# wangyunpeng139/3_ORB_SLAM3_SelfNote

Hardware: AMD Instinct MI355X
Metric: frames/sec ORB extract+match, 752x480 (higher is better)
Workload: dtype u8; 1 GPU; BASELINE configs[2]: extract + SearchByProjection match, 1000x1000 candidates, synthetic frame stream; image=752x480, nfeatures=1000, nlevels=8, batch=256, distinct_frames_per_gpu=2048, streams=4

## Files before the change

3_orb_slam3_selfnote_amd/csrc/orb_common.h:

```cpp
#pragma once
#include <stdint.h>
#include <stddef.h>

#define ORB_EDGE_THRESHOLD 19
#define ORB_PATCH_SIZE 31
#define ORB_HALF_PATCH 15
#define ORB_MIN_BORDER 16
#define ORB_DISC_PIXELS 749
#define ORB_MAXL 16

#define FAST_TILE_PITCH 80
#define FAST_TILE_COLS 65
#define FAST_TILE_ROWS 76
#define FAST_S_PITCH 64

#define FAST_REC_WORDS 32
#define FAST_REC_GROUP_WORDS 8
#define FAST_REC_CELL_WORDS 4

#ifndef ORB_DESCRIBE_K
#define ORB_DESCRIBE_K 8
#endif
#define ORB_DESCRIBE_GROUPS(totalKp, K) ((((totalKp) + (K) - 1) / (K) + 3) / 4 > 1 ? (((totalKp) + (K) - 1) / (K) + 3) / 4 : 1)

__host__ __device__ constexpr int clamp_count(int n, int cap) { return (n > 0 ? n : 0) < cap ? (n > 0 ? n : 0) : cap; }
static_assert(clamp_count(-1, 8) == 0 && clamp_count(0, 8) == 0 && clamp_count(5, 8) == 5 && clamp_count(8, 8) == 8 && clamp_count(9, 8) == 8, "clamp_count");
static_assert(clamp_count(-1, 0) == 0 && clamp_count(0, 0) == 0 && clamp_count(1, 0) == 0, "clamp_count: cap == 0");

struct LiveCount {
  const int32_t *dev; int stride; int konst;
  __device__ __forceinline__ int at(int p, int cap) const { return dev ? clamp_count(dev[(size_t)p * stride], cap) : konst; }
};

// ... 7 lines not shown
  int nCols, nRows, wCell, hCell;
  int cellCap;
  int cellBase;
  int slotBase;
  int N;
  int nIni;
  float hX;
  int candBase;
  int candCap;
  int kpBase, kpCap;
  float scale;
  float kpsize;
  int xtabBase, ytabBase;
  int resizeRows;
  int resizeSrcRows;
  int tilesX, tilesY, tileBase;
  uint32_t rowTileMagic;
};

#define CHAIN_TILE 32
#define CHAIN_NT 1024
struct ChainTile {
  uint16_t level, pad;
  uint16_t x[ORB_MAXL], y[ORB_MAXL], w[ORB_MAXL], h[ORB_MAXL];
};

struct FrameParams {
  LevelGeom geom[ORB_MAXL];
  int nlevels;
  int nframes;
// ... 8 lines not shown
  uint32_t *cand;    int cand_fs;
  uint16_t *knode;
  uint32_t *lkp;     int lkp_fs;
  uint16_t *lrank;
  int32_t *lcnt;
  int32_t *candCnt;
  const int2 *xtab, *ytab;
  const int8_t *disc;
  const uint32_t *tiles;
  uint32_t magicCells, magicTiles, magicKpBlk;
  int totalTiles;
  int totalCells;
  int totalGroups;
  uint32_t magicGroups;
  const uint32_t *fastRecs;
  int totalKp;
  int octCap;
  const ChainTile *chain;
  int chainBuf0, chainBuf1;
  void *out_kps;
  uint8_t *out_desc;
  int32_t *out_counts;
  int cap;
};
```

3_orb_slam3_selfnote_amd/csrc/orb_kernels.h:

```cpp
#pragma once
#include <hip/hip_runtime.h>
#include <type_traits>
#include "orb_common.h"
#include "orb_fast_score.h"
#include "orb_sincos.h"

#define WAVE 64

__constant__ __attribute__((aligned(16))) int8_t c_pattern[1024] = {
#include "../../include/orb_pattern_data.inc"
};

struct DiscTab { uint32_t w[64][6]; };
constexpr int kDiscUmax[16] = {15, 15, 15, 15, 14, 14, 14, 13, 13, 12, 11, 10, 9, 8, 6, 3};
constexpr DiscTab make_disc_tab() {
  DiscTab t{};
  int n = 0;
  for (int v = -15; v <= 15; v++) {
    const int d = kDiscUmax[v < 0 ? -v : v];
    for (int u = -d; u <= d; u++) {
      const int lane = n & 63, k = n >> 6;
      t.w[lane][k >> 2] |= (uint32_t)(uint8_t)(int8_t)u << (8 * (k & 3));
      t.w[lane][3 + (k >> 2)] |= (uint32_t)(uint8_t)(int8_t)v << (8 * (k & 3));
      n++;
// ... 77 lines not shown
    uint32_t inc = wave_incl_scan(v);
    if (lane == 63) sw[wid] = inc;
    __syncthreads();
    const uint32_t wsum = lane < NW ? sw[lane] : 0u;
    const uint32_t wincl = wave_incl_scan(wsum);
    const int widu = __builtin_amdgcn_readfirstlane(wid);
    const uint32_t woff = (uint32_t)__builtin_amdgcn_readlane((int)(wincl - wsum), widu);
    const uint32_t tot = (uint32_t)__builtin_amdgcn_readlane((int)wincl, NW - 1);
    if (i < n) a[i] = carry + woff + inc - v;
    carry += tot;
    __syncthreads();
  }
  return carry;
}

#define RESIZE_ROWS_MAX 16
#define RESIZE_MAXSRC 32
__global__ __launch_bounds__(256) void k_resize(FrameParams P, int level, int smemRowBytes, int tPitch, int maxSrc) {
  extern __shared__ __align__(16) uint8_t smem_rs[];
  const LevelGeom G = P.geom[level];
  const LevelGeom Gs = P.geom[level - 1];
  const int tid = threadIdx.x;
  int frame, rowTile;
  xcd_map((G.h + G.resizeRows - 1) / G.resizeRows, G.rowTileMagic, P.nframes, frame, rowTile);
  const int dy0 = rowTile * G.resizeRows;
  const int nrows = min(G.resizeRows, G.h - dy0);
  int spitch;
  const uint8_t *src = level_plane(P, frame, level - 1, spitch);
  uint8_t *dstplane = P.pyr + (size_t)frame * P.pyr_fs + G.off;
  const int wq = (G.w + 3) & ~3, qw = wq >> 2;
  __shared__ int2 sY[RESIZE_ROWS_MAX];
  if (tid < nrows) sY[tid] = P.ytab[G.ytabBase + dy0 + tid];

  if (tPitch > 0) {
    const int syFirst = min(max(P.ytab[G.ytabBase + dy0].x, 0), Gs.h - 1);
    const int syLast = min(max(P.ytab[G.ytabBase + dy0 + nrows - 1].x + 1, 0), Gs.h - 1);
    const int nsrc = min(syLast - syFirst + 1, maxSrc);
    uint8_t *sRows = smem_rs;
    uint8_t *sT = sRows + (size_t)maxSrc * smemRowBytes;
    uint4 *sRowRec = reinterpret_cast<uint4 *>(sT + (((size_t)maxSrc * tPitch + 15) & ~(size_t)15));
    const int4 *xtab4 = reinterpret_cast<const int4 *>(P.xtab + G.xtabBase);
    int4 xtPre[2];
#pragma unroll
    for (int k = 0; k < 2; k++) { const int p = tid + 256 * k; xtPre[k] = 2 * p < wq ? xtab4[p] : make_int4(0, 0, 0, 0); }
    const bool aligned = ((((uintptr_t)src) | (uintptr_t)spitch) & 3u) == 0;
    const uint8_t *src0 = src + (size_t)syFirst * spitch;
    if (aligned) {
      const int cpr = smemRowBytes >> 4, nfull = Gs.w >> 4;
      const float inv_cpr = 1.0f / (float)cpr;
      for (int idx = tid; idx < cpr * nsrc; idx += 256) {
        const int r = (int)(((float)idx + 0.5f) * inv_cpr), c = idx - (int)mul24((uint32_t)r, (uint32_t)cpr);
        if (c < nfull)
          __builtin_amdgcn_global_load_lds((const __attribute__((address_space(1))) void *)(src0 + (mul24((uint32_t)r, (uint32_t)spitch) + 16u * (uint32_t)c)),
                                           (__attribute__((address_space(3))) void *)(sRows + (size_t)(idx - (tid & 63)) * 16), 16, 0, 0);
      }
      const int ndw = (Gs.w + 3) >> 2, d0 = 4 * nfull, ntail = ndw - d0;
      const bool lastRowPartial = (Gs.w & 3) != 0;
      for (int idx = tid; idx < ntail * nsrc; idx += 256) {
        const int r = idx / ntail, d = d0 + (idx - r * ntail);
// ... 2 lines not shown
        if (lastRowPartial && d == ndw - 1 && syFirst + r == Gs.h - 1 && spitch < 4 * ndw) {
          v = 0;
          for (int b = 0; 4 * d + b < Gs.w; b++) v |= (uint32_t)rowp[4 * d + b] << (8 * b);
        } else {
          v = *reinterpret_cast<const uint32_t *>(rowp + 4 * d);
        }
        *reinterpret_cast<uint32_t *>(sRows + mul24((uint32_t)r, (uint32_t)smemRowBytes) + 4 * d) = v;
      }
    } else {
      const float inv_w = 1.0f / (float)Gs.w;
      for (int idx = tid; idx < Gs.w * nsrc; idx += 256) {
        const int r = (int)(((float)idx + 0.5f) * inv_w), c = idx - (int)mul24((uint32_t)r, (uint32_t)Gs.w);
        sRows[mul24((uint32_t)r, (uint32_t)smemRowBytes) + c] = src0[mul24((uint32_t)r, (uint32_t)spitch) + c];
      }
    }
    if (tid < nrows) {
      const int2 yt = P.ytab[G.ytabBase + dy0 + tid];
      const int sy0 = min(max(yt.x, 0), Gs.h - 1), sy1 = min(max(yt.x + 1, 0), Gs.h - 1);
      sRowRec[tid] = make_uint4((uint32_t)((sy0 - syFirst) * tPitch), (uint32_t)((sy1 - syFirst) * tPitch), (uint32_t)yt.y, (uint32_t)((dy0 + tid) * G.pitch));
    }
    __syncthreads();
    typedef unsigned short u16x2 __attribute__((ext_vector_type(2)));
    auto dot2 = [](uint32_t pix, uint32_t coef) -> uint32_t {
      u16x2 x, y;
      __builtin_memcpy(&x, &pix, 4); __builtin_memcpy(&y, &coef, 4);
      return __builtin_amdgcn_udot2(x, y, 0u, false);
    };
    int trip = 0;
    for (int p = tid; 2 * p < wq; p += 256, trip++) {
      const int4 xt = trip == 0 ? xtPre[0] : trip == 1 ? xtPre[1] : xtab4[p];
      const uint32_t base = (uint32_t)xt.x & ~3u, oA = (uint32_t)xt.x & 3u, oB = (uint32_t)xt.z - base;
      const uint32_t selA = 0x0c000c00u | oA | ((oA + 1u) << 16), selB = 0x0c000c00u | oB | ((oB + 1u) << 16);
      const uint32_t kA = (uint32_t)xt.y << 4, kB = (uint32_t)xt.w << 4;
      const uint8_t *sp = sRows + base;
      uint8_t *tp = sT + 4 * p;
      for (int r = 0; r < nsrc; r += 4) {
// ... 20 lines not shown
      for (int qx = tid & 31; qx < qw; qx += 32) {
        const uint2 t0 = *reinterpret_cast<const uint2 *>(T0 + 8 * qx), t1 = *reinterpret_cast<const uint2 *>(T1 + 8 * qx);
        const uint32_t u0[4] = {t0.x & 0xffffu, t0.x >> 16, t0.y & 0xffffu, t0.y >> 16};
        const uint32_t u1[4] = {t1.x & 0xffffu, t1.x >> 16, t1.y & 0xffffu, t1.y >> 16};
        uint32_t packed = 0;
#pragma unroll
        for (int j = 0; j < 4; j++) {
          const uint32_t v = ((mul24_vv(b0, u0[j]) >> 16) + (mul24_vv(b1, u1[j]) >> 16) + 2) >> 2;
          packed |= v << (8 * j);
        }
        const int dx0 = 4 * qx;
        if (dx0 + 3 < G.w) *reinterpret_cast<uint32_t *>(dst + dx0) = packed;
        else for (int j = 0; j < 4 && dx0 + j < G.w; j++) dst[dx0 + j] = (uint8_t)(packed >> (8 * j));
      }
    }
    return;
  }

  int2 *sX = reinterpret_cast<int2 *>(smem_rs);
  for (int i = tid; i < wq; i += 256) sX[i] = P.xtab[G.xtabBase + i];
  __syncthreads();
  const float inv_qw = 1.0f / (float)qw;
  for (int q = tid; q < qw * nrows; q += 256) {
    const int ry = (int)(((float)q + 0.5f) * inv_qw), dx0 = (q - (int)mul24((uint32_t)ry, (uint32_t)qw)) * 4, dy = dy0 + ry;
    const int2 yt = sY[ry];
    const int sy0 = min(max(yt.x, 0), Gs.h - 1), sy1 = min(max(yt.x + 1, 0), Gs.h - 1);
    const int b0 = yt.y & 0xffff, b1 = (yt.y >> 16) & 0xffff;
    const uint8_t *S0 = src + mul24((uint32_t)sy0, (uint32_t)spitch), *S1 = src + mul24((uint32_t)sy1, (uint32_t)spitch);
    uint32_t packed = 0;
#pragma unroll
    for (int j = 0; j < 4; j++) {
      const int2 xt = sX[dx0 + j];
      const int sx = xt.x, sx1 = min(sx + 1, Gs.w - 1);
      const int a0 = xt.y & 0xffff, a1 = (xt.y >> 16) & 0xffff;
      const int r0 = S0[sx] * a0 + S0[sx1] * a1;
      const int r1 = S1[sx] * a0 + S1[sx1] * a1;
      const int v = (((b0 * (r0 >> 4)) >> 16) + ((b1 * (r1 >> 4)) >> 16) + 2) >> 2;
      packed |= (uint32_t)v << (8 * j);
    }
    uint8_t *dst = dstplane + mul24((uint32_t)dy, (uint32_t)G.pitch);
    if (dx0 + 3 < G.w) *reinterpret_cast<uint32_t *>(dst + dx0) = packed;
    else for (int j = 0; j < 4 && dx0 + j < G.w; j++) dst[dx0 + j] = (uint8_t)(packed >> (8 * j));
  }
}

__global__ __launch_bounds__(CHAIN_NT) void k_pyramid_chain(FrameParams P) {
  extern __shared__ __align__(16) uint8_t smem_ch[];
  const int tid = threadIdx.x, lane = tid & 63, wid = tid >> 6;
  constexpr int NW = CHAIN_NT / 64;
  const int ntile = (int)gridDim.x / P.nframes;
  const int frame = (int)blockIdx.x / ntile, tile = (int)blockIdx.x - frame * ntile;
  __shared__ ChainTile T;
  static_assert(sizeof(ChainTile) % 4 == 0 && sizeof(ChainTile) / 4 <= CHAIN_NT, "one dword per thread");
  if (tid < (int)(sizeof(ChainTile) / 4)) reinterpret_cast<uint32_t *>(&T)[tid] = reinterpret_cast<const uint32_t *>(&P.chain[tile])[tid];
  __syncthreads();
  const int L = T.level;
  uint8_t *buf[2] = {smem_ch, smem_ch + P.chainBuf0};
  int2 *sTab = reinterpret_cast<int2 *>(smem_ch + P.chainBuf0 + P.chainBuf1);
// ... 53 lines not shown
  const int B = (int)(uint16_t)min((uint16_t)max(p0, p8), (uint16_t)max(p4, p12));
  return (D - (v - t)) | ((v + t) - B);
}

#ifndef FAST_NT
#define FAST_NT 256
#endif
#define FAST_QUEUE 128
#ifndef FAST_LIST
#define FAST_LIST 384
#endif
static_assert(FAST_NT == 4 * WAVE, "k_fast gives each cell of a 2 x 2 group a wavefront of its own");
static_assert(FAST_LIST % WAVE == 0, "pass 3 reads the corner list 64 entries at a time, all inside the list");
static_assert((FAST_TILE_ROWS * FAST_TILE_PITCH) % 16 == 0, "the score plane is cleared in 16-byte stores");
static_assert(FAST_TILE_ROWS * FAST_TILE_PITCH <= 65536, "queue entries are 16-bit tile offsets");
#if defined(FAST_STAMPS) || defined(OCT_STAMPS)
__device__ unsigned int *g_fast_stamps;
#endif
#ifdef FAST_STAMPS
#define FSTAMP(i) do { const long long t_ = __builtin_readcyclecounter(); if (threadIdx.x == 0 && g_fast_stamps) g_fast_stamps[(size_t)blockIdx.x * 8 + (i)] = (unsigned int)(t_ - ft0); ft0 = t_; } while (0)
#else
#define FSTAMP(i) do {} while (0)
#endif
__device__ __forceinline__ void wave_lds_order() {
  __builtin_amdgcn_wave_barrier();
  asm volatile("" ::: "memory");
}
__global__ __launch_bounds__(FAST_NT) void k_fast(FrameParams P) {
#ifdef FAST_STAMPS
  long long ft0 = __builtin_readcyclecounter();
#endif
  __shared__ __align__(16) uint8_t sTile[FAST_TILE_ROWS * FAST_TILE_PITCH];
  __shared__ __align__(16) uint8_t sS[FAST_TILE_ROWS * FAST_TILE_PITCH];
// ... 542 lines not shown
        t.v[lane][8 + 4 * s + d] = vv;
      }
  }
  return t;
}
__device__ const BlurTab g_blurTab = make_blur_tab();

#define BLUR_TX 128
#ifndef BLUR_TY
#define BLUR_TY 64
#endif
#define BLUR_ROWS_IN (BLUR_TY + 6)
#define BLURM_PITCH 176
#define BLURM_OPITCH 144
__global__ __launch_bounds__(256) __attribute__((amdgpu_waves_per_eu(7, 7))) void k_blur(FrameParams P) {
  typedef int v4i __attribute__((ext_vector_type(4)));
  typedef int v16i __attribute__((ext_vector_type(16)));
  __shared__ __align__(16) uint8_t sLds[BLUR_ROWS_IN * BLURM_PITCH + BLUR_TY * BLURM_OPITCH];
  static_assert(BLUR_TY % 32 == 0 && (BLUR_TY + 32) * BLURM_PITCH <= BLUR_ROWS_IN * BLURM_PITCH + BLUR_TY * BLURM_OPITCH, "the last block's rows must stay inside the allocation");
  uint8_t *sIn = sLds, *sOut = sLds + BLUR_ROWS_IN * BLURM_PITCH;
  const int tid = threadIdx.x, lane = tid & 63, wid = tid >> 6;
  int tile, frame;
  xcd_map(P.totalTiles, P.magicTiles, P.nframes, frame, tile);
  const uint4 t0 = reinterpret_cast<const uint4 *>(P.tiles)[2 * tile], t1 = reinterpret_cast<const uint4 *>(P.tiles)[2 * tile + 1];
  const int x0 = (int)(t0.x & 0xffffu), y0 = (int)(t0.x >> 16), level = (int)t0.y;
  struct { int w, h, bpitch; size_t boff; } G;
  G.w = (int)(t0.z & 0xffffu); G.h = (int)(t0.z >> 16); G.bpitch = (int)(t0.w >> 16);
  G.boff = ((size_t)t1.w << 32) | t1.z;
  int pitch;
  const uint8_t *img;
  if (level == 0) { pitch = (int)P.img0_stride; img = P.img0 + (size_t)frame * P.img0_frame_stride; }
  else { pitch = (int)(t0.w & 0xffffu); img = P.pyr + (size_t)frame * P.pyr_fs + (((size_t)t1.y << 32) | t1.x); }
  const bool aligned = ((((uintptr_t)img) | (uintptr_t)pitch) & 3u) == 0;
  const int wlim = level == 0 ? G.w : pitch;
  const bool dma = aligned && G.w >= 160 && G.h >= 40 && (wlim & 15) == 0;
  const bool edgeL = x0 == 0, edgeR = x0 + 131 >= G.w;
  if (dma) {
    for (int idx = tid; idx < BLUR_ROWS_IN * 11; idx += 256) {
      const uint32_t r = mul24((uint32_t)idx, 5958u) >> 16, c = (uint32_t)idx - 11u * r;
      int yy = y0 - 3 + (int)r;
      yy = yy < 0 ? -yy : yy;
      yy = yy >= G.h ? 2 * (G.h - 1) - yy : yy;
      yy = max(yy, 0);
      int xb = x0 - 16 + 16 * (int)c;
      xb = min(max(xb, 0), wlim - 16);
      __builtin_amdgcn_global_load_lds((const __attribute__((address_space(1))) void *)(img + (mul24((uint32_t)yy, (uint32_t)pitch) + (uint32_t)xb)),
                                       (__attribute__((address_space(3))) void *)(sIn + idx * 16), 16, 0, 0);
    }
    if (edgeL || edgeR) {
      __syncthreads();
      for (int i = tid; i < BLUR_ROWS_IN * 6; i += 256) {
        const int r = (int)(mul24((uint32_t)i, 10923u) >> 16), k = i - 6 * r;
        const int x = k < 3 ? -1 - k : G.w + (k - 3);
        const int xs = k < 3 ? 1 + k : G.w - 2 - (k - 3);
        const bool need = k < 3 ? edgeL : (edgeR && x - (x0 - 16) < 160);
        if (need) sIn[r * BLURM_PITCH + (x - (x0 - 16))] = sIn[r * BLURM_PITCH + (xs - (x0 - 16))];
      }
    }
  } else {
    const bool small = G.w < 16 || G.h < 16;
    auto srcRow = [&](int r) {
      int yy = y0 + r - 3;
      if (small) yy = reflect101(yy, G.h);
// ... 6 lines not shown
      const uint8_t *row = srcRow((int)r);
      uint32_t v;
      if (aligned && xb >= 0 && xb + 3 < G.w) v = *reinterpret_cast<const uint32_t *>(row + xb);
      else {
        v = 0;
#pragma unroll
        for (int kk = 0; kk < 4; kk++) {
          int xx = xb + kk;
          if (small) xx = reflect101(xx, G.w);
          else { xx = xx < 0 ? -xx : xx; xx = xx >= G.w ? 2 * (G.w - 1) - xx : xx; xx = max(xx, 0); }
          v |= (uint32_t)row[xx] << (8 * kk);
        }
      }
      *reinterpret_cast<uint32_t *>(sIn + r * BLURM_PITCH + 4u * c) = v;
    }
  }
  const int n = lane & 31, hh = lane >> 5;
  v4i Hb[2], Va[2];
  {
    const uint4 *tab = reinterpret_cast<const uint4 *>(g_blurTab.v[lane]);
    const uint4 q0 = tab[0], q1 = tab[1], q2 = tab[2], q3 = tab[3];
    Hb[0] = v4i{(int)q0.x, (int)q0.y, (int)q0.z, (int)q0.w}; Hb[1] = v4i{(int)q1.x, (int)q1.y, (int)q1.z, (int)q1.w};
    Va[0] = v4i{(int)q2.x, (int)q2.y, (int)q2.z, (int)q2.w}; Va[1] = v4i{(int)q3.x, (int)q3.y, (int)q3.z, (int)q3.w};
  }
  __syncthreads();
  auto row_sums = [&](int mt, v4i &Bhi, v4i &Blo) {
    int seedT = 128 * 257;
    asm volatile("" : "+v"(seedT));
    v16i acc;
#pragma unroll
    for (int j = 0; j < 16; j++) acc[j] = seedT;
#pragma unroll
    for (int s = 0; s < 2; s++) {
      v4i a = *reinterpret_cast<const v4i *>(sIn + (32 * mt + n) * BLURM_PITCH + 32 * wid + 32 * s + 16 * hh);
      a[0] ^= (int)0x80808080; a[1] ^= (int)0x80808080; a[2] ^= (int)0x80808080; a[3] ^= (int)0x80808080;
      acc = __builtin_amdgcn_mfma_i32_32x32x32_i8(a, Hb[s], acc, 0, 0, 0);
    }
#pragma unroll
    for (int d = 0; d < 4; d++) {
      const uint32_t p01 = __builtin_amdgcn_perm((uint32_t)acc[4 * d + 1], (uint32_t)acc[4 * d], 0x05010400u);
// ... 17 lines not shown
      sOut[(row0 + (j & 3) + 8 * (j >> 2) + 4 * hh) * BLURM_OPITCH + 32 * wid + n] = (uint8_t)b;
    }
  };
  v4i Hp, Lp, Hc, Lc;
  row_sums(0, Hp, Lp);
#pragma unroll
  for (int k = 0; k < BLUR_TY / 32; k++) {
    if (k > 0 && y0 + 32 * k >= G.h) break;
    __builtin_amdgcn_sched_barrier(0);
    row_sums(k + 1, Hc, Lc);
    __builtin_amdgcn_sched_barrier(0);
    outputs(Hp, Lp, Hc, Lc, 32 * k);
    Hp = Hc; Lp = Lc;
  }
  __syncthreads();
#pragma unroll
  for (int t = 0; t < BLUR_TY / 32; t++) {
    const int row = (tid >> 3) + 32 * t, seg = tid & 7;
    const int y = y0 + row, x = x0 + 16 * seg;
    if (y < G.h && x < G.w) {
      uint8_t *out = P.blur + (size_t)frame * P.blur_fs + G.boff + (size_t)y * G.bpitch + x;
      const uint4 v = *reinterpret_cast<const uint4 *>(sOut + row * BLURM_OPITCH + 16 * seg);
      if (x + 16 <= G.bpitch) *reinterpret_cast<uint4 *>(out) = v;
      else {
        const uint8_t *b = sOut + row * BLURM_OPITCH + 16 * seg;
        for (int cc = 0; cc < 16 && x + cc < G.w; cc++) out[cc] = b[cc];
      }
    }
  }
}

__device__ __forceinline__ float fast_atan2_deg(float y, float x) {
  const float scale = (float)(180.0 / 3.1415926535897932384626433832795);
  const float p1 = 0.9997878412794807f * scale, p3 = -0.3258083974640975f * scale;
  const float p5 = 0.1555786518463281f * scale, p7 = -0.04432655554792128f * scale;
  float ax = fabsf(x), ay = fabsf(y);
  float a, c, c2;
  if (ax >= ay) {
    c = ay / (ax + (float)2.2204460492503131e-16);
    c2 = c * c;
    a = (((p7 * c2 + p5) * c2 + p3) * c2 + p1) * c;
  } else {
    c = ax / (ay + (float)2.2204460492503131e-16);
    c2 = c * c;
// ... 696 lines not shown
```

3_orb_slam3_selfnote_amd/csrc/orbhip.hip:

```cpp
#include <hip/hip_runtime.h>
#include <math.h>
#include <cmath>
#include <assert.h>
#include <stdio.h>
#include <stdlib.h>
#include <string.h>
#include <string>
#include <vector>
#include <algorithm>
#include <type_traits>
#include <mutex>
#include <map>
#include <chrono>

#include "../../include/orbhip.h"
#include "orb_kernels.h"
#include "orb_match_kernels.h"
#include "orb_match_mfma.h"
#include "orb_project_kernels.h"
#include "orb_stereo_kernels.h"
#include "orb_depth_kernels.h"
#include "orb_rig_stereo_kernels.h"
#include "orb_newpoints_kernels.h"
#include "orb_fuse_kernels.h"
// ... 45 lines not shown
  int device = 0;
  int nfeatures = 0, nlevels = 0, iniThFAST = 0, minThFAST = 0;
  double scaleFactor = 0;
  std::vector<float> mvScaleFactor, mvInvScaleFactor, mvLevelSigma2, mvInvLevelSigma2;
  std::vector<int> mnFeaturesPerLevel;
  int umax[ORB_HALF_PATCH + 1];
  int rows = 0, cols = 0, max_batch = 0;
  std::vector<LevelGeom> geom;
  size_t pyr_fs = 0, blur_fs = 0, slot_fs = 0;
  bool octCellsLds = false;
  int chainTiles = 0, chainBuf0 = 0, chainBuf1 = 0;
  size_t chainLds = 0;
  size_t octLds = 0;
  int cell_fs = 0, cand_fs = 0, lkp_fs = 0, totalTiles = 0, totalCells = 0, totalGroups = 0, totalKp = 0, octCap = 0;
  int maxKeypoints = 0;
  DevBuf d_pyr, d_blur, d_cellCnt, d_cellOff, d_slots, d_cand, d_knode, d_lkp, d_lrank, d_lcnt, d_candCnt, d_fastRecs, d_tiles, d_xtab,
      d_ytab, d_disc, d_chain;
  DevBuf d_img, d_okps;
  hipStream_t stream = nullptr;
  float host_us[4] = {0, 0, 0, 0};
  FrameParams last{};
  bool have_last = false;
  hipEvent_t last_done = nullptr;
  bool last_pending = false;
  bool in_capture = false;
  DevBuf stereo[7];
  DevBuf stereo_batch[3];
  DevBuf maps[2];
  int maps_rows = 0, maps_cols = 0;
  void *pin_in = nullptr, *pin_out = nullptr;
  size_t pin_in_bytes = 0, pin_out_bytes = 0;
// ... 163 lines not shown
  if (hipStreamCreateWithFlags(&h->stream, hipStreamNonBlocking) != hipSuccess) { delete h; return nullptr; }
  if (h->d_disc.reserve(disc.size()) != hipSuccess ||
      copy_on(h->stream, h->d_disc.p, disc.data(), disc.size(), hipMemcpyHostToDevice) != hipSuccess) {
    (void)hipStreamDestroy(h->stream);
    delete h;
    return nullptr;
  }
  return h;
}

void orbx_destroy(orbx_t *h) {
  if (!h) return;
  (void)hipSetDevice(h->device);
  if (h->stream) (void)hipStreamSynchronize(h->stream);
  DevBuf *bufs[] = {&h->d_pyr, &h->d_blur, &h->d_cellCnt, &h->d_cellOff, &h->d_slots, &h->d_cand, &h->d_knode, &h->d_lkp,
                    &h->d_lrank, &h->d_lcnt, &h->d_candCnt, &h->d_fastRecs, &h->d_tiles, &h->d_xtab, &h->d_ytab, &h->d_disc, &h->d_chain, &h->d_img, &h->d_okps};
  for (DevBuf *b : bufs) b->release();
  for (DevBuf &b : h->stereo) b.release();
  for (DevBuf &b : h->stereo_batch) b.release();
  for (DevBuf &b : h->maps) b.release();
  if (h->graph) (void)hipGraphExecDestroy(h->graph);
  if (h->last_done) (void)hipEventDestroy(h->last_done);
  if (h->pin_in) (void)hipHostFree(h->pin_in);
  if (h->pin_pyr) (void)hipHostFree(h->pin_pyr);
  h->d_pyrpack.release();
  if (h->pin_out) (void)hipHostFree(h->pin_out);
  if (h->ev_ok)
    for (auto &set : h->ev)
      for (auto &e : set) (void)hipEventDestroy(e);
  if (h->stream) (void)hipStreamDestroy(h->stream);
  delete h;
// ... 10 lines not shown
    if (isf) isf[i] = h->mvInvScaleFactor[i];
    if (s2) s2[i] = h->mvLevelSigma2[i];
    if (is2) is2[i] = h->mvInvLevelSigma2[i];
  }
  return h->nlevels;
}

int orbx_get_features_per_level(const orbx_t *h, int *n) {
  if (!h || !n) return ORBX_E_ARG;
  for (int i = 0; i < h->nlevels; i++) n[i] = h->mnFeaturesPerLevel[i];
  return h->nlevels;
}

static uint32_t magic_div(uint32_t n) { return n <= 1 ? 0xffffffffu : (uint32_t)((1ull << 32) / n); }

#if defined(FAST_STAMPS) || defined(OCT_STAMPS)
int orbx_debug_fast_stamps(void *d_buf) {
  unsigned int *p = (unsigned int *)d_buf;
  return hipMemcpyToSymbol(HIP_SYMBOL(g_fast_stamps), &p, sizeof(p)) == hipSuccess ? 0 : -1;
}
#endif

int orbx_max_keypoints(const orbx_t *h) { return h ? h->maxKeypoints : ORBX_E_ARG; }

int orbx_configure(orbx_t *h, int rows, int cols, int max_batch) {
  if (!h || rows <= 0 || cols <= 0 || max_batch <= 0) return ORBX_E_ARG;
  if (rows > 4096 || cols > 4096) { h->err = "image larger than 4096x4096 (12-bit packed coordinates)"; return ORBX_E_ARG; }
  if (max_batch > 65535) { h->err = "batch larger than 65535"; return ORBX_E_ARG; }
  if (h->rows == rows && h->cols == cols && h->max_batch >= max_batch) return h->maxKeypoints;
  XCHECK(h, hipSetDevice(h->device));
  XCHECK(h, hipStreamSynchronize(h->stream));
  const int nl = h->nlevels;
  std::vector<LevelGeom> g(nl);
  std::vector<int2> xtab, ytab;
  size_t pyr = 0, blur = 0;
  int cells = 0, slots = 0, kps = 0, tiles = 0, octCap = 8;
  for (int l = 0; l < nl; l++) {
    LevelGeom &G = g[l];
    memset(&G, 0, sizeof(G));
    const float inv = h->mvInvScaleFactor[l];
    G.w = cv_round((float)cols * inv);
    G.h = cv_round((float)rows * inv);
    if (G.w < 1 || G.h < 1) { h->err = "pyramid level collapses to zero size"; return ORBX_E_ARG; }
    G.pitch = (int)align_up((size_t)G.w, 64);
    G.bpitch = G.pitch;
    G.off = pyr;
    if (l > 0) pyr += align_up((size_t)G.pitch * G.h, 256);
    G.boff = blur;
    blur += align_up((size_t)G.bpitch * G.h, 256);
// ... 63 lines not shown
        ytab.push_back(make_int2(sy, (b0 & 0xffff) | (b1 << 16)));
      }
      auto src_rows = [&](int rows) {
        int m = 0;
        for (int dy0 = 0; dy0 < G.h; dy0 += rows) {
          const int nrows = std::min(rows, G.h - dy0);
          const int f = std::min(std::max(ytab[G.ytabBase + dy0].x, 0), sh - 1), la = std::min(std::max(ytab[G.ytabBase + dy0 + nrows - 1].x + 1, 0), sh - 1);
          m = std::max(m, la - f + 1);
        }
        return m;
      };
      const size_t rowStage = align_up((size_t)sw + 4, 16) + align_up((size_t)((G.w + 3) & ~3) * 2, 8);
      G.resizeRows = RESIZE_ROWS_MAX;
      G.resizeSrcRows = src_rows(G.resizeRows);
      if ((size_t)G.resizeSrcRows * rowStage > 64 * 1024 || G.resizeSrcRows > RESIZE_MAXSRC) { G.resizeRows = 8; G.resizeSrcRows = src_rows(8); }
    } else { G.resizeRows = RESIZE_ROWS_MAX; G.resizeSrcRows = 0; }
  }
  if (slots > (1 << 30)) { h->err = "workspace too large"; return ORBX_E_ARG; }
  std::vector<uint32_t> cellrec((size_t)std::max(cells, 1) * 4, 0u);
  for (int l = 0; l < nl; l++) {
    LevelGeom &G = g[l];
    G.rowTileMagic = magic_div((uint32_t)((G.h + G.resizeRows - 1) / G.resizeRows));
    for (int ci = 0; ci < G.nRows; ci++)
      for (int cj = 0; cj < G.nCols; cj++) {
        const int c = ci * G.nCols + cj;
        uint32_t *R = &cellrec[(size_t)(G.cellBase + c) * 4];
        const int iniX = ORB_MIN_BORDER + cj * G.wCell, iniY = ORB_MIN_BORDER + ci * G.hCell;
        const int maxX = std::min(iniX + G.wCell + 6, G.maxBorderX), maxY = std::min(iniY + G.hCell + 6, G.maxBorderY);
        const int tw = maxX - iniX, th = maxY - iniY;
        const bool valid = !(iniX >= G.maxBorderX - 6 || iniY >= G.maxBorderY - 3 || tw - 6 <= 0 || th - 6 <= 0);
// ... 42 lines not shown
            C[1] = R[1];
            C[2] = R[2];
            C[3] = (uint32_t)cell;
          }
      }
  }
  h->totalGroups = (int)(grouprec.size() / FAST_REC_WORDS);
  std::vector<uint32_t> tilerec((size_t)std::max(tiles, 1) * 8, 0u);
  for (int l = 0; l < nl; l++) {
    const LevelGeom &G = g[l];
    if (G.pitch > 65535 || G.bpitch > 65535) { h->err = "level pitch above 65535"; return ORBX_E_ARG; }
    if (l > 0 && (size_t)((G.w + 3) & ~3) * 8 > ORB_LDS_LIMIT - 1024) { h->err = "pyramid level wider than 20000 columns"; return ORBX_E_ARG; }
    for (int ty = 0; ty < G.tilesY; ty++)
      for (int tx = 0; tx < G.tilesX; tx++) {
        uint32_t *R = &tilerec[(size_t)(G.tileBase + ty * G.tilesX + tx) * 8];
        R[0] = (uint32_t)(tx * BLUR_TX) | ((uint32_t)(ty * BLUR_TY) << 16);
        R[1] = (uint32_t)l;
        R[2] = (uint32_t)G.w | ((uint32_t)G.h << 16);
        R[3] = (uint32_t)G.pitch | ((uint32_t)G.bpitch << 16);
        R[4] = (uint32_t)(G.off & 0xffffffffu); R[5] = (uint32_t)((uint64_t)G.off >> 32);
        R[6] = (uint32_t)(G.boff & 0xffffffffu); R[7] = (uint32_t)((uint64_t)G.boff >> 32);
      }
  }
  h->geom = g;
  h->pyr_fs = std::max<size_t>(pyr, 256);
  h->blur_fs = blur;
  h->cell_fs = std::max(cells, 1);
  h->slot_fs = (size_t)std::max(slots, 1);
  h->cand_fs = std::max(slots, 1);
  h->lkp_fs = kps;
  h->totalTiles = tiles;
  h->totalCells = cells;
// ... 2 lines not shown
  h->maxKeypoints = kps;
  const size_t B = (size_t)max_batch;
  XCHECK(h, h->d_pyr.reserve(h->pyr_fs * B));
  XCHECK(h, h->d_blur.reserve(h->blur_fs * B));
  XCHECK(h, h->d_cellCnt.reserve(sizeof(uint32_t) * h->cell_fs * B));
  XCHECK(h, h->d_cellOff.reserve(sizeof(uint32_t) * h->cell_fs * B));
  XCHECK(h, h->d_slots.reserve(sizeof(uint32_t) * h->slot_fs * B));
  XCHECK(h, h->d_cand.reserve(sizeof(uint32_t) * (size_t)h->cand_fs * B));
  XCHECK(h, h->d_knode.reserve(sizeof(uint16_t) * (size_t)h->cand_fs * B));
  XCHECK(h, h->d_lkp.reserve(sizeof(uint32_t) * (size_t)h->lkp_fs * B));
  XCHECK(h, h->d_lrank.reserve(sizeof(uint16_t) * (size_t)h->lkp_fs * B));
  XCHECK(h, h->d_lcnt.reserve(sizeof(int32_t) * 2 * nl * B));
  XCHECK(h, h->d_candCnt.reserve(sizeof(int32_t) * nl * B));
  XCHECK(h, h->d_fastRecs.reserve(sizeof(uint32_t) * std::max<size_t>(grouprec.size(), FAST_REC_WORDS)));
  if (!grouprec.empty()) XCHECK(h, copy_on(h->stream, h->d_fastRecs.p, grouprec.data(), sizeof(uint32_t) * grouprec.size(), hipMemcpyHostToDevice));
  XCHECK(h, h->d_tiles.reserve(sizeof(uint32_t) * tilerec.size()));
  XCHECK(h, copy_on(h->stream, h->d_tiles.p, tilerec.data(), sizeof(uint32_t) * tilerec.size(), hipMemcpyHostToDevice));
  XCHECK(h, h->d_xtab.reserve(sizeof(int2) * std::max<size_t>(xtab.size(), 1)));
  XCHECK(h, h->d_ytab.reserve(sizeof(int2) * std::max<size_t>(ytab.size(), 1)));
  if (!xtab.empty()) XCHECK(h, copy_on(h->stream, h->d_xtab.p, xtab.data(), sizeof(int2) * xtab.size(), hipMemcpyHostToDevice));
  if (!ytab.empty()) XCHECK(h, copy_on(h->stream, h->d_ytab.p, ytab.data(), sizeof(int2) * ytab.size(), hipMemcpyHostToDevice));
  {
    std::vector<ChainTile> tilesC;
    size_t b0 = 0, b1 = 0, tabMax = 0;
    for (int L = nl - 1; L >= 1; L--)
      for (int ty = 0; ty < g[L].h; ty += CHAIN_TILE)
        for (int tx = 0; tx < g[L].w; tx += CHAIN_TILE) {
          ChainTile T;
          memset(&T, 0, sizeof(T));
          T.level = (uint16_t)L;
// ... 104 lines not shown
  P.blur = (uint8_t *)h->d_blur.p;     P.blur_fs = h->blur_fs;
  P.cellCnt = (uint32_t *)h->d_cellCnt.p; P.cell_fs = h->cell_fs;
  P.slots = (uint32_t *)h->d_slots.p;  P.slot_fs = h->slot_fs;
  P.cand = (uint32_t *)h->d_cand.p;    P.cand_fs = h->cand_fs;
  P.knode = (uint16_t *)h->d_knode.p;
  P.lkp = (uint32_t *)h->d_lkp.p;      P.lkp_fs = h->lkp_fs;
  P.lrank = (uint16_t *)h->d_lrank.p;
  P.lcnt = (int32_t *)h->d_lcnt.p;
  P.candCnt = (int32_t *)h->d_candCnt.p;
  P.xtab = (const int2 *)h->d_xtab.p;
  P.ytab = (const int2 *)h->d_ytab.p;
  P.disc = (const int8_t *)h->d_disc.p;
  P.totalTiles = h->totalTiles;
  P.totalCells = h->totalCells;
  P.fastRecs = (const uint32_t *)h->d_fastRecs.p;
  P.totalGroups = h->totalGroups;
  P.magicGroups = magic_div((uint32_t)std::max(h->totalGroups, 1));
  P.tiles = (const uint32_t *)h->d_tiles.p;
  P.magicCells = magic_div((uint32_t)std::max(h->totalCells, 1));
  P.magicTiles = magic_div((uint32_t)std::max(h->totalTiles, 1));
  const bool wide = (long long)h->nlevels * nframes <= 32;
  const int describeGroups = wide ? ORB_DESCRIBE_GROUPS(h->totalKp, 1) : ORB_DESCRIBE_GROUPS(h->totalKp, ORB_DESCRIBE_K);
  P.magicKpBlk = magic_div((uint32_t)describeGroups);
  P.totalKp = h->totalKp;
  P.octCap = h->octCap;
  P.chain = (const ChainTile *)h->d_chain.p; P.chainBuf0 = h->chainBuf0; P.chainBuf1 = h->chainBuf1;
  P.out_kps = d_kps;
  P.out_desc = d_desc;
  P.out_counts = d_counts;
  P.cap = cap;
  const bool prof = h->profiling && h->ev_ok;
  hipEvent_t *pev = h->ev[h->prof_head % PROF_DEPTH];
  if (prof) XCHECK(h, hipEventRecord(pev[0], s));
  const bool printForms = getenv("ORBHIP_PRINT_EXTRACT_FORMS") != nullptr;
  std::string pyrForm = h->nlevels == 1 ? "none" : "";
  if (wide && h->chainTiles > 0) { hipLaunchKernelGGL(k_pyramid_chain, dim3(h->chainTiles * nframes), dim3(CHAIN_NT), h->chainLds, s, P); pyrForm = "chain"; }
  else
  for (int l = 1; l < h->nlevels; l++) {
    const LevelGeom &G = h->geom[l], &Gs = h->geom[l - 1];
    const int rowBytes = (int)align_up((size_t)Gs.w + 4, 16);
    const int wq = (G.w + 3) & ~3;
    const int tPitch2 = (int)align_up((size_t)wq * 2, 8);
    const size_t lds2 = (size_t)G.resizeSrcRows * rowBytes + align_up((size_t)G.resizeSrcRows * tPitch2, 16) + 16 * RESIZE_ROWS_MAX;
    const bool twoPass = G.resizeSrcRows <= RESIZE_MAXSRC && (double)Gs.w / G.w < 3.0 && lds2 <= ORB_LDS_LIMIT - 1024;
    const int tPitch = twoPass ? tPitch2 : 0;
    const size_t lds = twoPass ? lds2 : (size_t)wq * 8;
    hipLaunchKernelGGL(k_resize, dim3(((G.h + G.resizeRows - 1) / G.resizeRows) * nframes), dim3(256), lds, s, P, l, rowBytes, tPitch, G.resizeSrcRows);
    if (printForms) pyrForm += std::string(l > 1 ? "," : "") + (!twoPass ? "1p" : G.resizeRows == 16 ? "2p16" : "2p8");
  }
  if (prof) XCHECK(h, hipEventRecord(pev[1], s));
  if (h->totalGroups > 0) hipLaunchKernelGGL(k_fast, dim3(h->totalGroups * nframes), dim3(FAST_NT), 0, s, P);
  if (prof) XCHECK(h, hipEventRecord(pev[2], s));
  if (wide) {
    if (h->octCellsLds) hipLaunchKernelGGL((k_octree<1024, true>), dim3(h->nlevels * nframes), dim3(1024), h->octLds, s, P, (uint32_t *)h->d_cellOff.p);
    else hipLaunchKernelGGL((k_octree<1024, false>), dim3(h->nlevels * nframes), dim3(1024), h->octLds, s, P, (uint32_t *)h->d_cellOff.p);
  } else {
    if (h->octCellsLds) hipLaunchKernelGGL((k_octree<256, true>), dim3(h->nlevels * nframes), dim3(256), h->octLds, s, P, (uint32_t *)h->d_cellOff.p);
    else hipLaunchKernelGGL((k_octree<256, false>), dim3(h->nlevels * nframes), dim3(256), h->octLds, s, P, (uint32_t *)h->d_cellOff.p);
  }
  if (prof) XCHECK(h, hipEventRecord(pev[3], s));
  hipLaunchKernelGGL(k_blur, dim3(h->totalTiles * nframes), dim3(256), 0, s, P);
// ... 4147 lines not shown
```

Measured before the change: 301,000 frames/s.

## Precompute resize row records and blur tile interior flags on host

Adds host-built per-row-tile records for the two-pass resize kernel (source row range, per-row LDS offsets, weights, destination offsets), loaded via global_load_lds, replacing per-block ytab reads and arithmetic. Blur tile records gain interior and whole-store flags so interior tiles take a simpler unclamped DMA load loop and skip per-store bounds checks. Blur coefficient loads are hoisted before the barrier to overlap with the async loads. Optional cycle-stamp instrumentation is added behind TILE_STAMPS; it costs extra device memory for records and more code paths.

Measured after the change: 307,300 frames/s, median of 6. +2.1%, better.

```diff
diff --git a/3_orb_slam3_selfnote_amd/csrc/orb_common.h b/3_orb_slam3_selfnote_amd/csrc/orb_common.h
--- a/3_orb_slam3_selfnote_amd/csrc/orb_common.h
+++ b/3_orb_slam3_selfnote_amd/csrc/orb_common.h
@@ -17,6 +17,13 @@
 #define FAST_REC_WORDS 32
 #define FAST_REC_GROUP_WORDS 8
 #define FAST_REC_CELL_WORDS 4
+
+#define RESIZE_ROWS_MAX 16
+#define RESIZE_REC_GROUP_WORDS 4
+#define RESIZE_REC_WORDS (RESIZE_REC_GROUP_WORDS + 4 * RESIZE_ROWS_MAX)
+
+#define BLUR_TILE_INTERIOR 0x100u
+#define BLUR_TILE_WHOLE_STORES 0x200u
 
 #ifndef ORB_DESCRIBE_K
 #define ORB_DESCRIBE_K 8
@@ -54,6 +61,8 @@
   int xtabBase, ytabBase;
   int resizeRows;
   int resizeSrcRows;
+  int resizeTPitch;
+  int resizeRecBase;
   int tilesX, tilesY, tileBase;
   uint32_t rowTileMagic;
 };
@@ -92,6 +101,7 @@
   int totalGroups;
   uint32_t magicGroups;
   const uint32_t *fastRecs;
+  const uint32_t *resizeRecs;
   int totalKp;
   int octCap;
   const ChainTile *chain;
diff --git a/3_orb_slam3_selfnote_amd/csrc/orb_kernels.h b/3_orb_slam3_selfnote_amd/csrc/orb_kernels.h
--- a/3_orb_slam3_selfnote_amd/csrc/orb_kernels.h
+++ b/3_orb_slam3_selfnote_amd/csrc/orb_kernels.h
@@ -115,28 +115,42 @@
   return carry;
 }
 
-#define RESIZE_ROWS_MAX 16
 #define RESIZE_MAXSRC 32
+#if defined(FAST_STAMPS) || defined(OCT_STAMPS) || defined(TILE_STAMPS)
+__device__ unsigned int *g_fast_stamps;
+#endif
+#ifdef TILE_STAMPS
+#define TSTAMP_BEGIN() const long long ts0_ = __builtin_readcyclecounter()
+#define TSTAMP(i, rowExpr, lvl) do { const long long t_ = __builtin_readcyclecounter(); if (threadIdx.x == 0 && g_fast_stamps) { const size_t r_ = (rowExpr); g_fast_stamps[r_ * 8 + (i)] = (unsigned int)(t_ - ts0_); g_fast_stamps[r_ * 8 + 3] = (unsigned int)((lvl) + 1); } } while (0)
+__device__ __forceinline__ size_t resize_stamp_row(const FrameParams &P, int level) {
+  size_t row = (size_t)P.totalTiles * P.nframes + blockIdx.x;
+  for (int l = 1; l < level; l++) row += (size_t)((P.geom[l].h + P.geom[l].resizeRows - 1) / P.geom[l].resizeRows) * P.nframes;
+  return row;
+}
+#else
+#define TSTAMP_BEGIN() do {} while (0)
+#define TSTAMP(i, rowExpr, lvl) do {} while (0)
+#endif
+#define RSTAMP(i) TSTAMP(i, resize_stamp_row(P, level), level)
 __global__ __launch_bounds__(256) void k_resize(FrameParams P, int level, int smemRowBytes, int tPitch, int maxSrc) {
+  TSTAMP_BEGIN();
   extern __shared__ __align__(16) uint8_t smem_rs[];
   const LevelGeom G = P.geom[level];
   const LevelGeom Gs = P.geom[level - 1];
   const int tid = threadIdx.x;
   int frame, rowTile;
   xcd_map((G.h + G.resizeRows - 1) / G.resizeRows, G.rowTileMagic, P.nframes, frame, rowTile);
-  const int dy0 = rowTile * G.resizeRows;
-  const int nrows = min(G.resizeRows, G.h - dy0);
   int spitch;
   const uint8_t *src = level_plane(P, frame, level - 1, spitch);
   uint8_t *dstplane = P.pyr + (size_t)frame * P.pyr_fs + G.off;
   const int wq = (G.w + 3) & ~3, qw = wq >> 2;
-  __shared__ int2 sY[RESIZE_ROWS_MAX];
-  if (tid < nrows) sY[tid] = P.ytab[G.ytabBase + dy0 + tid];
+  const uint32_t *tileRec = P.resizeRecs + (size_t)(G.resizeRecBase + rowTile) * RESIZE_REC_WORDS;
 
   if (tPitch > 0) {
-    const int syFirst = min(max(P.ytab[G.ytabBase + dy0].x, 0), Gs.h - 1);
-    const int syLast = min(max(P.ytab[G.ytabBase + dy0 + nrows - 1].x + 1, 0), Gs.h - 1);
-    const int nsrc = min(syLast - syFirst + 1, maxSrc);
+    typedef uint32_t rec4_t __attribute__((ext_vector_type(4)));
+    const __attribute__((address_space(4))) uint32_t *rec = (const __attribute__((address_space(4))) uint32_t *)tileRec;
+    const rec4_t gr = *reinterpret_cast<const __attribute__((address_space(4))) rec4_t *>(rec);
+    const int syFirst = (int)gr[0], nsrc = (int)gr[1], nrows = (int)gr[2];
     uint8_t *sRows = smem_rs;
     uint8_t *sT = sRows + (size_t)maxSrc * smemRowBytes;
     uint4 *sRowRec = reinterpret_cast<uint4 *>(sT + (((size_t)maxSrc * tPitch + 15) & ~(size_t)15));
@@ -144,6 +158,9 @@
     int4 xtPre[2];
 #pragma unroll
     for (int k = 0; k < 2; k++) { const int p = tid + 256 * k; xtPre[k] = 2 * p < wq ? xtab4[p] : make_int4(0, 0, 0, 0); }
+    if (tid < nrows)
+      __builtin_amdgcn_global_load_lds((const __attribute__((address_space(1))) void *)(tileRec + RESIZE_REC_GROUP_WORDS + 4 * tid),
+                                       (__attribute__((address_space(3))) void *)sRowRec, 16, 0, 0);
     const bool aligned = ((((uintptr_t)src) | (uintptr_t)spitch) & 3u) == 0;
     const uint8_t *src0 = src + (size_t)syFirst * spitch;
     if (aligned) {
@@ -176,12 +193,9 @@
         sRows[mul24((uint32_t)r, (uint32_t)smemRowBytes) + c] = src0[mul24((uint32_t)r, (uint32_t)spitch) + c];
       }
     }
-    if (tid < nrows) {
-      const int2 yt = P.ytab[G.ytabBase + dy0 + tid];
-      const int sy0 = min(max(yt.x, 0), Gs.h - 1), sy1 = min(max(yt.x + 1, 0), Gs.h - 1);
-      sRowRec[tid] = make_uint4((uint32_t)((sy0 - syFirst) * tPitch), (uint32_t)((sy1 - syFirst) * tPitch), (uint32_t)yt.y, (uint32_t)((dy0 + tid) * G.pitch));
-    }
-    __syncthreads();
+    RSTAMP(0);
+    __syncthreads();
+    RSTAMP(1);
     typedef unsigned short u16x2 __attribute__((ext_vector_type(2)));
     auto dot2 = [](uint32_t pix, uint32_t coef) -> uint32_t {
       u16x2 x, y;
@@ -232,9 +246,14 @@
         else for (int j = 0; j < 4 && dx0 + j < G.w; j++) dst[dx0 + j] = (uint8_t)(packed >> (8 * j));
       }
     }
+    RSTAMP(2);
     return;
   }
 
+  const int dy0 = rowTile * G.resizeRows;
+  const int nrows = min(G.resizeRows, G.h - dy0);
+  __shared__ int2 sY[RESIZE_ROWS_MAX];
+  if (tid < nrows) sY[tid] = P.ytab[G.ytabBase + dy0 + tid];
   int2 *sX = reinterpret_cast<int2 *>(smem_rs);
   for (int i = tid; i < wq; i += 256) sX[i] = P.xtab[G.xtabBase + i];
   __syncthreads();
@@ -260,6 +279,7 @@
     if (dx0 + 3 < G.w) *reinterpret_cast<uint32_t *>(dst + dx0) = packed;
     else for (int j = 0; j < 4 && dx0 + j < G.w; j++) dst[dx0 + j] = (uint8_t)(packed >> (8 * j));
   }
+  RSTAMP(2);
 }
 
 __global__ __launch_bounds__(CHAIN_NT) void k_pyramid_chain(FrameParams P) {
@@ -343,9 +363,6 @@
 static_assert(FAST_LIST % WAVE == 0, "pass 3 reads the corner list 64 entries at a time, all inside the list");
 static_assert((FAST_TILE_ROWS * FAST_TILE_PITCH) % 16 == 0, "the score plane is cleared in 16-byte stores");
 static_assert(FAST_TILE_ROWS * FAST_TILE_PITCH <= 65536, "queue entries are 16-bit tile offsets");
-#if defined(FAST_STAMPS) || defined(OCT_STAMPS)
-__device__ unsigned int *g_fast_stamps;
-#endif
 #ifdef FAST_STAMPS
 #define FSTAMP(i) do { const long long t_ = __builtin_readcyclecounter(); if (threadIdx.x == 0 && g_fast_stamps) g_fast_stamps[(size_t)blockIdx.x * 8 + (i)] = (unsigned int)(t_ - ft0); ft0 = t_; } while (0)
 #else
@@ -918,6 +935,8 @@
 #define BLURM_PITCH 176
 #define BLURM_OPITCH 144
 __global__ __launch_bounds__(256) __attribute__((amdgpu_waves_per_eu(7, 7))) void k_blur(FrameParams P) {
+#define BSTAMP(i) TSTAMP(i, (size_t)blockIdx.x, level)
+  TSTAMP_BEGIN();
   typedef int v4i __attribute__((ext_vector_type(4)));
   typedef int v16i __attribute__((ext_vector_type(16)));
   __shared__ __align__(16) uint8_t sLds[BLUR_ROWS_IN * BLURM_PITCH + BLUR_TY * BLURM_OPITCH];
@@ -927,7 +946,8 @@
   int tile, frame;
   xcd_map(P.totalTiles, P.magicTiles, P.nframes, frame, tile);
   const uint4 t0 = reinterpret_cast<const uint4 *>(P.tiles)[2 * tile], t1 = reinterpret_cast<const uint4 *>(P.tiles)[2 * tile + 1];
-  const int x0 = (int)(t0.x & 0xffffu), y0 = (int)(t0.x >> 16), level = (int)t0.y;
+  const int x0 = (int)(t0.x & 0xffffu), y0 = (int)(t0.x >> 16), level = (int)(t0.y & 0xffu);
+  const bool interior = (t0.y & BLUR_TILE_INTERIOR) != 0u, wholeStores = (t0.y & BLUR_TILE_WHOLE_STORES) != 0u;
   struct { int w, h, bpitch; size_t boff; } G;
   G.w = (int)(t0.z & 0xffffu); G.h = (int)(t0.z >> 16); G.bpitch = (int)(t0.w >> 16);
   G.boff = ((size_t)t1.w << 32) | t1.z;
@@ -939,7 +959,30 @@
   const int wlim = level == 0 ? G.w : pitch;
   const bool dma = aligned && G.w >= 160 && G.h >= 40 && (wlim & 15) == 0;
   const bool edgeL = x0 == 0, edgeR = x0 + 131 >= G.w;
-  if (dma) {
+  const int n = lane & 31, hh = lane >> 5;
+  v4i Hb[2], Va[2];
+  {
+    const uint4 *tab = reinterpret_cast<const uint4 *>(g_blurTab.v[lane]);
+    const uint4 q0 = tab[0], q1 = tab[1], q2 = tab[2], q3 = tab[3];
+    Hb[0] = v4i{(int)q0.x, (int)q0.y, (int)q0.z, (int)q0.w}; Hb[1] = v4i{(int)q1.x, (int)q1.y, (int)q1.z, (int)q1.w};
+    Va[0] = v4i{(int)q2.x, (int)q2.y, (int)q2.z, (int)q2.w}; Va[1] = v4i{(int)q3.x, (int)q3.y, (int)q3.z, (int)q3.w};
+  }
+  if (dma && interior) {
+    const uint8_t *tile0 = img + ((uint32_t)(y0 - 3) * (uint32_t)pitch + (uint32_t)(x0 - 16));
+    const uint32_t r0 = mul24((uint32_t)tid, 5958u) >> 16;
+    uint32_t c = (uint32_t)tid - 11u * r0, off = mul24(r0, (uint32_t)pitch) + 16u * c;
+    const uint32_t step = 23u * (uint32_t)pitch + 48u, stepWrap = 24u * (uint32_t)pitch - 128u;
+#pragma unroll
+    for (int k = 0; k < (BLUR_ROWS_IN * 11 + 255) / 256; k++) {
+      if (256 * (k + 1) <= BLUR_ROWS_IN * 11 || tid + 256 * k < BLUR_ROWS_IN * 11)
+        __builtin_amdgcn_global_load_lds((const __attribute__((address_space(1))) void *)(tile0 + off),
+                                         (__attribute__((address_space(3))) void *)(sIn + (tid + 256 * k) * 16), 16, 0, 0);
+      const bool wrap = c >= 8u;
+      c = wrap ? c - 8u : c + 3u;
+      off += wrap ? stepWrap : step;
+    }
+    BSTAMP(0);
+  } else if (dma) {
     for (int idx = tid; idx < BLUR_ROWS_IN * 11; idx += 256) {
       const uint32_t r = mul24((uint32_t)idx, 5958u) >> 16, c = (uint32_t)idx - 11u * r;
       int yy = y0 - 3 + (int)r;
@@ -951,6 +994,7 @@
       __builtin_amdgcn_global_load_lds((const __attribute__((address_space(1))) void *)(img + (mul24((uint32_t)yy, (uint32_t)pitch) + (uint32_t)xb)),
                                        (__attribute__((address_space(3))) void *)(sIn + idx * 16), 16, 0, 0);
     }
+    BSTAMP(0);
     if (edgeL || edgeR) {
       __syncthreads();
       for (int i = tid; i < BLUR_ROWS_IN * 6; i += 256) {
@@ -987,16 +1031,10 @@
       }
       *reinterpret_cast<uint32_t *>(sIn + r * BLURM_PITCH + 4u * c) = v;
     }
-  }
-  const int n = lane & 31, hh = lane >> 5;
-  v4i Hb[2], Va[2];
-  {
-    const uint4 *tab = reinterpret_cast<const uint4 *>(g_blurTab.v[lane]);
-    const uint4 q0 = tab[0], q1 = tab[1], q2 = tab[2], q3 = tab[3];
-    Hb[0] = v4i{(int)q0.x, (int)q0.y, (int)q0.z, (int)q0.w}; Hb[1] = v4i{(int)q1.x, (int)q1.y, (int)q1.z, (int)q1.w};
-    Va[0] = v4i{(int)q2.x, (int)q2.y, (int)q2.z, (int)q2.w}; Va[1] = v4i{(int)q3.x, (int)q3.y, (int)q3.z, (int)q3.w};
-  }
-  __syncthreads();
+    BSTAMP(0);
+  }
+  __syncthreads();
+  BSTAMP(1);
   auto row_sums = [&](int mt, v4i &Bhi, v4i &Blo) {
     int seedT = 128 * 257;
     asm volatile("" : "+v"(seedT));
@@ -1044,20 +1082,26 @@
     Hp = Hc; Lp = Lc;
   }
   __syncthreads();
-#pragma unroll
-  for (int t = 0; t < BLUR_TY / 32; t++) {
-    const int row = (tid >> 3) + 32 * t, seg = tid & 7;
-    const int y = y0 + row, x = x0 + 16 * seg;
-    if (y < G.h && x < G.w) {
-      uint8_t *out = P.blur + (size_t)frame * P.blur_fs + G.boff + (size_t)y * G.bpitch + x;
-      const uint4 v = *reinterpret_cast<const uint4 *>(sOut + row * BLURM_OPITCH + 16 * seg);
-      if (x + 16 <= G.bpitch) *reinterpret_cast<uint4 *>(out) = v;
-      else {
-        const uint8_t *b = sOut + row * BLURM_OPITCH + 16 * seg;
-        for (int cc = 0; cc < 16 && x + cc < G.w; cc++) out[cc] = b[cc];
-      }
-    }
-  }
+  {
+    uint8_t *out0 = P.blur + (size_t)frame * P.blur_fs + G.boff + (size_t)y0 * G.bpitch + x0;
+    const int row = tid >> 3, seg = tid & 7, x = x0 + 16 * seg;
+    const uint8_t *b = sOut + row * BLURM_OPITCH + 16 * seg;
+    uint32_t off = mul24((uint32_t)row, (uint32_t)G.bpitch) + 16u * (uint32_t)seg;
+#pragma unroll
+    for (int t = 0; t < BLUR_TY / 32; t++) {
+      if (y0 + row + 32 * t < G.h && x < G.w) {
+        if (wholeStores || x + 16 <= G.bpitch) *reinterpret_cast<uint4 *>(out0 + off) = *reinterpret_cast<const uint4 *>(b);
+        else {
+#pragma clang loop vectorize(disable) unroll(disable)
+          for (int cc = 0; cc < 16 && x + cc < G.w; cc++) out0[off + cc] = b[cc];
+        }
+      }
+      b += 32 * BLURM_OPITCH;
+      off += 32u * (uint32_t)G.bpitch;
+    }
+  }
+  BSTAMP(2);
+#undef BSTAMP
 }
 
 __device__ __forceinline__ float fast_atan2_deg(float y, float x) {
diff --git a/3_orb_slam3_selfnote_amd/csrc/orbhip.hip b/3_orb_slam3_selfnote_amd/csrc/orbhip.hip
--- a/3_orb_slam3_selfnote_amd/csrc/orbhip.hip
+++ b/3_orb_slam3_selfnote_amd/csrc/orbhip.hip
@@ -83,7 +83,7 @@
   size_t octLds = 0;
   int cell_fs = 0, cand_fs = 0, lkp_fs = 0, totalTiles = 0, totalCells = 0, totalGroups = 0, totalKp = 0, octCap = 0;
   int maxKeypoints = 0;
-  DevBuf d_pyr, d_blur, d_cellCnt, d_cellOff, d_slots, d_cand, d_knode, d_lkp, d_lrank, d_lcnt, d_candCnt, d_fastRecs, d_tiles, d_xtab,
+  DevBuf d_pyr, d_blur, d_cellCnt, d_cellOff, d_slots, d_cand, d_knode, d_lkp, d_lrank, d_lcnt, d_candCnt, d_fastRecs, d_resizeRecs, d_tiles, d_xtab,
       d_ytab, d_disc, d_chain;
   DevBuf d_img, d_okps;
   hipStream_t stream = nullptr;
@@ -277,7 +277,7 @@
   (void)hipSetDevice(h->device);
   if (h->stream) (void)hipStreamSynchronize(h->stream);
   DevBuf *bufs[] = {&h->d_pyr, &h->d_blur, &h->d_cellCnt, &h->d_cellOff, &h->d_slots, &h->d_cand, &h->d_knode, &h->d_lkp,
-                    &h->d_lrank, &h->d_lcnt, &h->d_candCnt, &h->d_fastRecs, &h->d_tiles, &h->d_xtab, &h->d_ytab, &h->d_disc, &h->d_chain, &h->d_img, &h->d_okps};
+                    &h->d_lrank, &h->d_lcnt, &h->d_candCnt, &h->d_fastRecs, &h->d_resizeRecs, &h->d_tiles, &h->d_xtab, &h->d_ytab, &h->d_disc, &h->d_chain, &h->d_img, &h->d_okps};
   for (DevBuf *b : bufs) b->release();
   for (DevBuf &b : h->stereo) b.release();
   for (DevBuf &b : h->stereo_batch) b.release();
@@ -318,7 +318,7 @@
 
 static uint32_t magic_div(uint32_t n) { return n <= 1 ? 0xffffffffu : (uint32_t)((1ull << 32) / n); }
 
-#if defined(FAST_STAMPS) || defined(OCT_STAMPS)
+#if defined(FAST_STAMPS) || defined(OCT_STAMPS) || defined(TILE_STAMPS)
 int orbx_debug_fast_stamps(void *d_buf) {
   unsigned int *p = (unsigned int *)d_buf;
   return hipMemcpyToSymbol(HIP_SYMBOL(g_fast_stamps), &p, sizeof(p)) == hipSuccess ? 0 : -1;
@@ -326,6 +326,16 @@
 #endif
 
 int orbx_max_keypoints(const orbx_t *h) { return h ? h->maxKeypoints : ORBX_E_ARG; }
+
+static int resize_form(const LevelGeom &G, const LevelGeom &Gs, size_t *lds) {
+  const int rowBytes = (int)align_up((size_t)Gs.w + 4, 16);
+  const int wq = (G.w + 3) & ~3;
+  const int tPitch2 = (int)align_up((size_t)wq * 2, 8);
+  const size_t lds2 = (size_t)G.resizeSrcRows * rowBytes + align_up((size_t)G.resizeSrcRows * tPitch2, 16) + 16 * RESIZE_ROWS_MAX;
+  const bool twoPass = G.resizeSrcRows <= RESIZE_MAXSRC && (double)Gs.w / G.w < 3.0 && lds2 <= ORB_LDS_LIMIT - 1024;
+  *lds = twoPass ? lds2 : (size_t)wq * 8;
+  return twoPass ? tPitch2 : 0;
+}
 
 int orbx_configure(orbx_t *h, int rows, int cols, int max_batch) {
   if (!h || rows <= 0 || cols <= 0 || max_batch <= 0) return ORBX_E_ARG;
@@ -337,6 +347,7 @@
   const int nl = h->nlevels;
   std::vector<LevelGeom> g(nl);
   std::vector<int2> xtab, ytab;
+  std::vector<uint32_t> resizerec;
   size_t pyr = 0, blur = 0;
   int cells = 0, slots = 0, kps = 0, tiles = 0, octCap = 8;
   for (int l = 0; l < nl; l++) {
@@ -430,6 +441,28 @@
       G.resizeRows = RESIZE_ROWS_MAX;
       G.resizeSrcRows = src_rows(G.resizeRows);
       if ((size_t)G.resizeSrcRows * rowStage > 64 * 1024 || G.resizeSrcRows > RESIZE_MAXSRC) { G.resizeRows = 8; G.resizeSrcRows = src_rows(8); }
+      size_t ldsUnused;
+      G.resizeTPitch = resize_form(G, g[l - 1], &ldsUnused);
+      G.resizeRecBase = (int)(resizerec.size() / RESIZE_REC_WORDS);
+      for (int dy0 = 0; dy0 < G.h; dy0 += G.resizeRows) {
+        const int nrows = std::min(G.resizeRows, G.h - dy0);
+        const int2 *yt = &ytab[G.ytabBase + dy0];
+        const int syFirst = std::min(std::max(yt[0].x, 0), sh - 1), syLast = std::min(std::max(yt[nrows - 1].x + 1, 0), sh - 1);
+        resizerec.resize(resizerec.size() + RESIZE_REC_WORDS, 0u);
+        uint32_t *Q = &resizerec[resizerec.size() - RESIZE_REC_WORDS];
+        Q[0] = (uint32_t)syFirst;
+        Q[1] = (uint32_t)std::min(syLast - syFirst + 1, G.resizeSrcRows);
+        Q[2] = (uint32_t)nrows;
+        Q[3] = (uint32_t)dy0;
+        for (int r = 0; r < nrows; r++) {
+          const int sy0 = std::min(std::max(yt[r].x, 0), sh - 1), sy1 = std::min(std::max(yt[r].x + 1, 0), sh - 1);
+          uint32_t *R = Q + RESIZE_REC_GROUP_WORDS + 4 * r;
+          R[0] = (uint32_t)((sy0 - syFirst) * G.resizeTPitch);
+          R[1] = (uint32_t)((sy1 - syFirst) * G.resizeTPitch);
+          R[2] = (uint32_t)yt[r].y;
+          R[3] = (uint32_t)((dy0 + r) * G.pitch);
+        }
+      }
     } else { G.resizeRows = RESIZE_ROWS_MAX; G.resizeSrcRows = 0; }
   }
   if (slots > (1 << 30)) { h->err = "workspace too large"; return ORBX_E_ARG; }
@@ -502,8 +535,13 @@
     for (int ty = 0; ty < G.tilesY; ty++)
       for (int tx = 0; tx < G.tilesX; tx++) {
         uint32_t *R = &tilerec[(size_t)(G.tileBase + ty * G.tilesX + tx) * 8];
-        R[0] = (uint32_t)(tx * BLUR_TX) | ((uint32_t)(ty * BLUR_TY) << 16);
-        R[1] = (uint32_t)l;
+        const int x0 = tx * BLUR_TX, y0 = ty * BLUR_TY;
+        const int wlim = l == 0 ? G.w : G.pitch;
+        const bool interior = y0 - 3 >= 0 && y0 + BLUR_TY + 2 < G.h && x0 - 16 >= 0 && x0 + 160 <= wlim && x0 + 131 < G.w;
+        bool whole = true;
+        for (int x = x0; x < std::min(x0 + BLUR_TX, G.w); x += 16) whole = whole && x + 16 <= G.bpitch;
+        R[0] = (uint32_t)x0 | ((uint32_t)y0 << 16);
+        R[1] = (uint32_t)l | (interior ? BLUR_TILE_INTERIOR : 0u) | (whole ? BLUR_TILE_WHOLE_STORES : 0u);
         R[2] = (uint32_t)G.w | ((uint32_t)G.h << 16);
         R[3] = (uint32_t)G.pitch | ((uint32_t)G.bpitch << 16);
         R[4] = (uint32_t)(G.off & 0xffffffffu); R[5] = (uint32_t)((uint64_t)G.off >> 32);
@@ -536,6 +574,8 @@
   XCHECK(h, h->d_candCnt.reserve(sizeof(int32_t) * nl * B));
   XCHECK(h, h->d_fastRecs.reserve(sizeof(uint32_t) * std::max<size_t>(grouprec.size(), FAST_REC_WORDS)));
   if (!grouprec.empty()) XCHECK(h, copy_on(h->stream, h->d_fastRecs.p, grouprec.data(), sizeof(uint32_t) * grouprec.size(), hipMemcpyHostToDevice));
+  XCHECK(h, h->d_resizeRecs.reserve(sizeof(uint32_t) * std::max<size_t>(resizerec.size(), RESIZE_REC_WORDS)));
+  if (!resizerec.empty()) XCHECK(h, copy_on(h->stream, h->d_resizeRecs.p, resizerec.data(), sizeof(uint32_t) * resizerec.size(), hipMemcpyHostToDevice));
   XCHECK(h, h->d_tiles.reserve(sizeof(uint32_t) * tilerec.size()));
   XCHECK(h, copy_on(h->stream, h->d_tiles.p, tilerec.data(), sizeof(uint32_t) * tilerec.size(), hipMemcpyHostToDevice));
   XCHECK(h, h->d_xtab.reserve(sizeof(int2) * std::max<size_t>(xtab.size(), 1)));
@@ -670,6 +710,7 @@
   P.totalTiles = h->totalTiles;
   P.totalCells = h->totalCells;
   P.fastRecs = (const uint32_t *)h->d_fastRecs.p;
+  P.resizeRecs = (const uint32_t *)h->d_resizeRecs.p;
   P.totalGroups = h->totalGroups;
   P.magicGroups = magic_div((uint32_t)std::max(h->totalGroups, 1));
   P.tiles = (const uint32_t *)h->d_tiles.p;
@@ -695,12 +736,10 @@
   for (int l = 1; l < h->nlevels; l++) {
     const LevelGeom &G = h->geom[l], &Gs = h->geom[l - 1];
     const int rowBytes = (int)align_up((size_t)Gs.w + 4, 16);
-    const int wq = (G.w + 3) & ~3;
-    const int tPitch2 = (int)align_up((size_t)wq * 2, 8);
-    const size_t lds2 = (size_t)G.resizeSrcRows * rowBytes + align_up((size_t)G.resizeSrcRows * tPitch2, 16) + 16 * RESIZE_ROWS_MAX;
-    const bool twoPass = G.resizeSrcRows <= RESIZE_MAXSRC && (double)Gs.w / G.w < 3.0 && lds2 <= ORB_LDS_LIMIT - 1024;
-    const int tPitch = twoPass ? tPitch2 : 0;
-    const size_t lds = twoPass ? lds2 : (size_t)wq * 8;
+    size_t lds;
+    (void)resize_form(G, Gs, &lds);
+    const int tPitch = G.resizeTPitch;
+    const bool twoPass = tPitch > 0;
     hipLaunchKernelGGL(k_resize, dim3(((G.h + G.resizeRows - 1) / G.resizeRows) * nframes), dim3(256), lds, s, P, l, rowBytes, tPitch, G.resizeSrcRows);
     if (printForms) pyrForm += std::string(l > 1 ? "," : "") + (!twoPass ? "1p" : G.resizeRows == 16 ? "2p16" : "2p8");
   }
```
